# gchq/annchor

Measured on AMD Instinct MI355X. Metric: knn_graph_builds_per_s (1 / Annchor.fit() wall-clock; BASELINE: k-NN graph build time + recall@k), higher is better.
Workload: dtype int32 bit-vectors (Levenshtein) + f64 (bounds/regression/selection); 1 GPU; load_strings Levenshtein N=1600 n_anchors=15 k=25 p_work=0.12 niters=2; parallelism=one GPU

## Files before the change

annchor_amd/csrc/select.hip:

```cpp
#include "common.h"
#include "rowsel.h"
#include "selstate.h"

__global__ __launch_bounds__(ROW_THREADS) void k_row_thresh(const int64_t *__restrict__ Iptr, RowSrc src, uint32_t k,
                                                           double *__restrict__ thresh, int cap)
{
    __shared__ RowSelShared sh;
    __shared__ RowCand rc;
    extern __shared__ __attribute__((aligned(16))) unsigned char dyn_rt[];
    uint64_t *keys = reinterpret_cast<uint64_t *>(dyn_rt);
    const int64_t i = row_of_block(gridDim.x);
    const int64_t b = Iptr[i];
    const int len = (int)(Iptr[i + 1] - b);
    if (len <= 0) { if (threadIdx.x == 0) thresh[i] = -INFINITY; return; }
    const RowView rv = row_view(src, i, b);
    const uint32_t kk = k >= (uint32_t)len ? (uint32_t)len - 1 : k;
    {
        const int cnt = row_candidates(rc, len, (int)kk + 1, [&](int s) { return ann_key_asc(rv.val(s)); }, [](int) { return true; },
                                       [](int, uint64_t, bool) {});
        const int cnts = cnt > (int)kk ? row_cand_shrink(rc, cnt, (int)kk + 1, src.shrink_min) : -1;
        if (cnts > (int)kk) {
            for (int e = threadIdx.x; e < cnts; e += ROW_THREADS) {
                const uint64_t ke = rc.key[e];
                uint32_t less = 0, leq = 0;
// ... 601 lines not shown
__host__ __device__ __forceinline__ unsigned long long ann_tie_scramble(int64_t p)
{
    return ((unsigned long long)p * 0x9E3779B97F4A7C15ull) >> 11;
}

#define TIE_HB 12
#define TIE_BINS (1 << TIE_HB)
#define TIE_SHIFT (53 - TIE_HB)
#define TIE_U 8
__global__ __launch_bounds__(256) void k_tie_hist(const double *__restrict__ prob, int64_t n, CutState *__restrict__ cs,
                                                 uint32_t *__restrict__ ghist )
{
    __shared__ uint32_t h[2][TIE_BINS];
    __shared__ unsigned long long acc[4];
    for (int t = threadIdx.x; t < 2 * TIE_BINS; t += 256) (&h[0][0])[t] = 0;
    if (threadIdx.x < 4) acc[threadIdx.x] = 0;
    __syncthreads();
    const double t1 = cs->t1, t5 = cs->t5;
    const bool need1 = !cs->all1, need5 = !cs->all5;
    unsigned long long g1 = 0, g5 = 0, n1 = 0, n5 = 0;
    const int64_t stride = (int64_t)gridDim.x * blockDim.x * TIE_U;
    for (int64_t p0 = (int64_t)blockIdx.x * blockDim.x * TIE_U + threadIdx.x; p0 < n; p0 += stride) {
        double v[TIE_U];
#pragma unroll
        for (int e = 0; e < TIE_U; ++e) v[e] = ann_ldc(prob, p0 + (int64_t)e * blockDim.x, n);
#pragma unroll
        for (int e = 0; e < TIE_U; ++e) {
            const int64_t p = p0 + (int64_t)e * blockDim.x;
            if (p >= n || !(v[e] >= 0.0)) continue;
            g1 += v[e] > t1;
            g5 += v[e] > t5;
            const bool m1 = need1 && v[e] == t1, m5 = need5 && v[e] == t5;
            if (m1 || m5) {
                const uint32_t bin = (uint32_t)(ann_tie_scramble(p) >> TIE_SHIFT);
                if (m1) { atomicAdd(&h[0][bin], 1u); ++n1; }
                if (m5) { atomicAdd(&h[1][bin], 1u); ++n5; }
            }
        }
    }
#pragma unroll
    for (int off = 32; off > 0; off >>= 1) {
        g1 += __shfl_xor(g1, off); g5 += __shfl_xor(g5, off); n1 += __shfl_xor(n1, off); n5 += __shfl_xor(n5, off);
    }
    if ((threadIdx.x & 63) == 0) { atomicAdd(&acc[0], g1); atomicAdd(&acc[1], g5); atomicAdd(&acc[2], n1); atomicAdd(&acc[3], n5); }
    __syncthreads();
    for (int t = threadIdx.x; t < 2 * TIE_BINS; t += 256) {
        const uint32_t c = (&h[0][0])[t];
        if (c) atomicAdd(&ghist[t], c);
    }
    if (threadIdx.x == 0) {
        if (acc[0]) atomicAdd((unsigned long long *)&cs->tie_gt1, acc[0]);
        if (acc[1]) atomicAdd((unsigned long long *)&cs->tie_gt5, acc[1]);
        if (acc[2]) atomicAdd((unsigned long long *)&cs->tie_n1, acc[2]);
        if (acc[3]) atomicAdd((unsigned long long *)&cs->tie_n5, acc[3]);
    }
}

__global__ __launch_bounds__(1024) void k_tie_pick(CutState *__restrict__ cs, uint32_t *__restrict__ ghist)
{
    __shared__ unsigned long long wsum[16];
    const int lane = threadIdx.x & 63, wave = threadIdx.x >> 6;
    for (int q = 0; q < 2; ++q) {
        const bool all = q == 0 ? cs->all1 : cs->all5;
        const long long cnt = q == 0 ? cs->tie_n1 : cs->tie_n5;
        const long long e = q == 0 ? cs->K1 - cs->tie_gt1 : cs->K5 - cs->tie_gt5;
        uint32_t *h = ghist + q * TIE_BINS;
        constexpr int PER = TIE_BINS / 1024;
        unsigned long long c[PER], mine = 0;
#pragma unroll
        for (int j = 0; j < PER; ++j) { c[j] = h[threadIdx.x * PER + j]; h[threadIdx.x * PER + j] = 0; mine += c[j]; }
        unsigned long long inc = mine;
#pragma unroll
        for (int off = 1; off < 64; off <<= 1) { const unsigned long long up = __shfl_up(inc, off); if (lane >= off) inc += up; }
        __syncthreads();
        if (lane == 63) wsum[wave] = inc;
        __syncthreads();
        unsigned long long before = inc - mine;
        for (int w2 = 0; w2 < wave; ++w2) before += wsum[w2];
        if (threadIdx.x == 0) {
            unsigned long long rk = ~0ull;
            long long bin = -1;
            if (!all && e < cnt) { if (e <= 0) rk = 0ull; else bin = -2; }
            if (q == 0) { cs->rk1 = rk; cs->tie_bin1 = bin; } else { cs->rk5 = rk; cs->tie_bin5 = bin; }
        }
        __syncthreads();
        if (!all && e < cnt && e > 0 && (long long)before < e && (long long)(before + mine) >= e) {
            long long accb = (long long)before;
#pragma unroll
            for (int j = 0; j < PER; ++j) {
                if (accb < e && accb + (long long)c[j] >= e) {
                    if (q == 0) { cs->tie_bin1 = threadIdx.x * PER + j; cs->tie_rem1 = e - accb; cs->tie_len1 = (long long)c[j]; }
                    else { cs->tie_bin5 = threadIdx.x * PER + j; cs->tie_rem5 = e - accb; cs->tie_len5 = (long long)c[j]; }
                }
                accb += (long long)c[j];
            }
        }
        __syncthreads();
    }
}

#define TIE_LCAP 1024
__global__ __launch_bounds__(256) void k_tie_collect(const double *__restrict__ prob, int64_t n, CutState *__restrict__ cs,
                                                    unsigned long long *__restrict__ list1, unsigned long long *__restrict__ list5,
                                                    long long cap)
{
    __shared__ unsigned long long lbuf[2][TIE_LCAP];
    __shared__ uint32_t lcnt[2];
    __shared__ unsigned long long lbase[2];
    const long long b1 = cs->tie_bin1, b5 = cs->tie_bin5;
    if (b1 < 0 && b5 < 0) return;
    if (threadIdx.x < 2) lcnt[threadIdx.x] = 0;
    __syncthreads();
    const double t1 = cs->t1, t5 = cs->t5;
    auto put = [&](int q, unsigned long long kk) {
        const uint32_t o = atomicAdd(&lcnt[q], 1u);
        if (o < TIE_LCAP) lbuf[q][o] = kk;
        else {
            const unsigned long long g = atomicAdd((unsigned long long *)(q == 0 ? &cs->tie_got1 : &cs->tie_got5), 1ull);
            if ((long long)g < cap) (q == 0 ? list1 : list5)[g] = kk;
        }
    };
    const int64_t stride = (int64_t)gridDim.x * blockDim.x * TIE_U;
    for (int64_t p0 = (int64_t)blockIdx.x * blockDim.x * TIE_U + threadIdx.x; p0 < n; p0 += stride) {
        double v[TIE_U];
#pragma unroll
        for (int e = 0; e < TIE_U; ++e) v[e] = ann_ldc(prob, p0 + (int64_t)e * blockDim.x, n);
#pragma unroll
        for (int e = 0; e < TIE_U; ++e) {
            const int64_t p = p0 + (int64_t)e * blockDim.x;
            if (p >= n || !(v[e] >= 0.0)) continue;
            const bool m1 = b1 >= 0 && v[e] == t1, m5 = b5 >= 0 && v[e] == t5;
            if (m1 || m5) {
                const unsigned long long kk = ann_tie_scramble(p);
                const long long bin = (long long)(kk >> TIE_SHIFT);
                if (m1 && bin == b1) put(0, kk);
                if (m5 && bin == b5) put(1, kk);
            }
        }
    }
    __syncthreads();
    if (threadIdx.x < 2) {
        const uint32_t m = min(lcnt[threadIdx.x], (uint32_t)TIE_LCAP);
        lbase[threadIdx.x] = m ? atomicAdd((unsigned long long *)(threadIdx.x == 0 ? &cs->tie_got1 : &cs->tie_got5), (unsigned long long)m) : 0ull;
    }
    __syncthreads();
    for (int q = 0; q < 2; ++q) {
        const uint32_t m = min(lcnt[q], (uint32_t)TIE_LCAP);
        unsigned long long *list = q == 0 ? list1 : list5;
        for (uint32_t t = threadIdx.x; t < m; t += blockDim.x)
            if ((long long)(lbase[q] + t) < cap) list[lbase[q] + t] = lbuf[q][t];
    }
}

__global__ __launch_bounds__(1024) void k_tie_select(CutState *__restrict__ cs, const unsigned long long *__restrict__ list1,
                                                    const unsigned long long *__restrict__ list5, long long cap)
{
    __shared__ uint32_t hist[256];
    __shared__ unsigned long long prefix_s;
    __shared__ long long krem_s;
    for (int q = 0; q < 2; ++q) {
        const long long bin = q == 0 ? cs->tie_bin1 : cs->tie_bin5;
        if (bin < 0) continue;
        const long long cnt = q == 0 ? cs->tie_len1 : cs->tie_len5;
        const long long e = q == 0 ? cs->tie_rem1 : cs->tie_rem5;
        const unsigned long long *list = q == 0 ? list1 : list5;
        unsigned long long rk = 0ull;
        if (cnt > cap) { if (threadIdx.x == 0) cs->tie_overflow = 1; }
        else {
            if (threadIdx.x == 0) { prefix_s = 0; krem_s = e - 1; }
            __syncthreads();
            for (int pass = 1; pass < 8; ++pass) {
                const int shift = 56 - 8 * pass;
                const unsigned long long himask = ~0ull << (shift + 8);
                if (threadIdx.x < 256) hist[threadIdx.x] = 0;
                __syncthreads();
                const unsigned long long pre = prefix_s;
                for (long long t = threadIdx.x; t < cnt; t += 1024) {
                    const unsigned long long kk = list[t];
                    if ((kk & himask) == pre) atomicAdd(&hist[(uint32_t)(kk >> shift) & 0xffu], 1u);
                }
                __syncthreads();
                if (threadIdx.x < 64) {
                    uint32_t c4[4], s4 = 0;
#pragma unroll
                    for (int j = 0; j < 4; ++j) { c4[j] = hist[threadIdx.x * 4 + j]; s4 += c4[j]; }
                    uint32_t inc = s4;
#pragma unroll
                    for (int off = 1; off < 64; off <<= 1) { const uint32_t up = __shfl_up(inc, off); if ((int)threadIdx.x >= off) inc += up; }
                    long long k = krem_s;
                    long long acc4 = (long long)(inc - s4);
                    if (acc4 <= k && k < acc4 + (long long)s4) {
#pragma unroll
                        for (int j = 0; j < 4; ++j) {
                            if (acc4 <= k && k < acc4 + (long long)c4[j]) {
                                prefix_s = pre | ((unsigned long long)(threadIdx.x * 4 + j) << shift);
                                krem_s = k - acc4;
                            }
                            acc4 += c4[j];
                        }
                    }
                }
                __syncthreads();
            }
            rk = prefix_s;
        }
        if (threadIdx.x == 0) { if (q == 0) cs->rk1 = rk; else cs->rk5 = rk; }
        __syncthreads();
    }
}

__global__ void k_tie_flags(const double *__restrict__ prob, int64_t n, double t, uint8_t *__restrict__ flag, double *__restrict__ scr)
{
    const int64_t p = (int64_t)blockIdx.x * blockDim.x + threadIdx.x;
    if (p < n) {
        flag[p] = prob[p] == t ? 1 : 0;
        scr[p] = (double)ann_tie_scramble(p);
    }
}

__device__ __forceinline__ int cut_class(double v, double t, unsigned long long rk, const double *RA, int64_t p)
{
    if (v > t) return 2;
    if (v != t) return 0;
    if (rk == ~0ull) return 2;
    const unsigned long long kk = ann_tie_scramble(p);
    return kk < rk ? 2 : (kk == rk ? 1 : 0);
}

__global__ __launch_bounds__(CP_THREADS) void k_cut_count(const double *__restrict__ prob, const double *__restrict__ RA, int64_t n,
                                                         const CutState *__restrict__ cs, uint32_t *__restrict__ blk, int nsub)
{
    __shared__ uint32_t acc[4];
    if (threadIdx.x < 4) acc[threadIdx.x] = 0;
    __syncthreads();
    const double t1 = cs->t1, t5 = cs->t5;
    const unsigned long long rk1 = cs->rk1, rk5 = cs->rk5;
    uint32_t g1 = 0, q1 = 0, g5 = 0, q5 = 0;
    for (int sub = 0; sub < nsub; ++sub) {
        const int64_t base = ((int64_t)blockIdx.x * nsub + sub) * CP_SUBTILE;
        if (base >= n) break;
        double v[CP_ITEMS];
#pragma unroll
        for (int k = 0; k < CP_ITEMS; ++k) v[k] = ann_ldc(prob, base + (int64_t)k * CP_THREADS + threadIdx.x, n);
#pragma unroll
        for (int k = 0; k < CP_ITEMS; ++k) {
            const int64_t p = base + (int64_t)k * CP_THREADS + threadIdx.x;
            if (p < n && v[k] >= 0.0) {
                const int c1 = cut_class(v[k], t1, rk1, RA, p), c5 = cut_class(v[k], t5, rk5, RA, p);
                g1 += c1 == 2; q1 += c1 == 1; g5 += c5 == 2; q5 += c5 == 1;
            }
        }
    }
    unsigned long long pk = (unsigned long long)g1 | ((unsigned long long)q1 << 16) | ((unsigned long long)g5 << 32) |
                            ((unsigned long long)q5 << 48);
#pragma unroll
    for (int off = 32; off > 0; off >>= 1) pk += __shfl_xor(pk, off);
    if ((threadIdx.x & 63) == 0) {
        atomicAdd(&acc[0], (uint32_t)(pk & 0xffff)); atomicAdd(&acc[1], (uint32_t)((pk >> 16) & 0xffff));
        atomicAdd(&acc[2], (uint32_t)((pk >> 32) & 0xffff)); atomicAdd(&acc[3], (uint32_t)(pk >> 48));
    }
    __syncthreads();
    if (threadIdx.x < 4) blk[(size_t)blockIdx.x * 4 + threadIdx.x] = acc[threadIdx.x];
}

#define CS_THREADS 1024
#define CS_ITEMS 4
__global__ __launch_bounds__(CS_THREADS) void k_cut_scan(const uint32_t *__restrict__ blk, int nb, CutState *__restrict__ cs,
                                                        int64_t *__restrict__ off)
{
    __shared__ unsigned long long wsum[CS_THREADS / 64];
    const int lane = threadIdx.x & 63, wave = threadIdx.x >> 6;
    auto block_scan = [&](unsigned long long v, unsigned long long *total) -> unsigned long long {
        unsigned long long inc = v;
#pragma unroll
        for (int o = 1; o < 64; o <<= 1) { unsigned long long x = __shfl_up(inc, o); if (lane >= o) inc += x; }
        __syncthreads();
        if (lane == 63) wsum[wave] = inc;
        __syncthreads();
        unsigned long long base = 0, tot = 0;
        for (int w = 0; w < CS_THREADS / 64; ++w) { const unsigned long long x = wsum[w]; if (w < wave) base += x; tot += x; }
        *total = tot;
        return base + inc - v;
    };
    const uint4 *blk4 = reinterpret_cast<const uint4 *>(blk);
    unsigned long long g = 0;
    for (int t0 = threadIdx.x; t0 < nb; t0 += CS_THREADS * CS_ITEMS) {
        uint4 b[CS_ITEMS];
#pragma unroll
        for (int e = 0; e < CS_ITEMS; ++e) b[e] = ann_ldc(blk4, t0 + e * CS_THREADS, nb);
#pragma unroll
        for (int e = 0; e < CS_ITEMS; ++e)
            if (t0 + e * CS_THREADS < nb) g += (unsigned long long)b[e].x | ((unsigned long long)b[e].z << 32);
    }
    unsigned long long T;
    block_scan(g, &T);
    const int64_t T1 = (int64_t)(T & 0xffffffffull), T5 = (int64_t)(T >> 32);
    const int64_t e1 = cs->all1 ? (1ll << 62) : cs->K1 - T1;
    const int64_t e5 = cs->all5 ? (1ll << 62) : cs->K5 - T5;
    const bool both_all = cs->all1 && cs->all5;
    unsigned long long c_eq = 0, c_out = 0;
    for (int base = 0; base < nb; base += CS_THREADS * CS_ITEMS) {
        const int t0 = base + threadIdx.x * CS_ITEMS;
        uint4 b[CS_ITEMS];
#pragma unroll
        for (int e = 0; e < CS_ITEMS; ++e) {
            b[e] = ann_ldc(blk4, t0 + e, nb);
            if (t0 + e >= nb) b[e] = make_uint4(0, 0, 0, 0);
        }
        unsigned long long eqs = 0;
#pragma unroll
        for (int e = 0; e < CS_ITEMS; ++e) eqs += (unsigned long long)b[e].y | ((unsigned long long)b[e].w << 32);
        unsigned long long tot;
        unsigned long long ex = c_eq + block_scan(eqs, &tot);
        c_eq += tot;
        int64_t p1[CS_ITEMS], p5[CS_ITEMS];
        unsigned long long outv[CS_ITEMS], outs = 0;
#pragma unroll
        for (int e = 0; e < CS_ITEMS; ++e) {
            p1[e] = (int64_t)(ex & 0xffffffffull);
            p5[e] = (int64_t)(ex >> 32);
            const int64_t eq1 = b[e].y, eq5 = b[e].w;
            const int64_t take1 = min(eq1, max((int64_t)0, e1 - p1[e]));
            const int64_t take5 = min(eq5, max((int64_t)0, e5 - p5[e]));
            const int64_t ncand = (int64_t)b[e].x + take1;
            const int64_t nbig = (int64_t)b[e].z + take5;
            const int64_t nnext = both_all ? nbig : nbig - ncand;
            outv[e] = (unsigned long long)ncand | ((unsigned long long)nnext << 32);
            outs += outv[e];
            ex += (unsigned long long)eq1 | ((unsigned long long)eq5 << 32);
        }
        unsigned long long exo = c_out + block_scan(outs, &tot);
        c_out += tot;
#pragma unroll
        for (int e = 0; e < CS_ITEMS; ++e) {
            if (t0 + e < nb) {
                int64_t *o = off + (size_t)(t0 + e) * 4;
                o[0] = p1[e]; o[1] = p5[e]; o[2] = (int64_t)(exo & 0xffffffffull); o[3] = (int64_t)(exo >> 32);
            }
            exo += outv[e];
        }
    }
    if (threadIdx.x == 0) { cs->e1 = e1; cs->e5 = e5; cs->ncand = (int64_t)(c_out & 0xffffffffull); cs->nnext = (int64_t)(c_out >> 32); }
}

__global__ __launch_bounds__(CP_THREADS) void k_cut_emit(const double *__restrict__ prob, const double *__restrict__ RA, int64_t n,
                                                        const CutState *__restrict__ cs, const int64_t *__restrict__ off,
                                                        int32_t *__restrict__ cand, int32_t *__restrict__ next, int nsub)
{
    __shared__ uint32_t wsum[CP_THREADS / 64];
    const double t1 = cs->t1, t5 = cs->t5;
    const unsigned long long rk1 = cs->rk1, rk5 = cs->rk5;
    const int64_t e1 = cs->e1, e5 = cs->e5;
    const bool both_all = cs->all1 && cs->all5;
    auto scan2 = [&](uint32_t a, uint32_t b, uint32_t *ea, uint32_t *eb, uint32_t *ta, uint32_t *tb) {
        uint32_t tot;
        const uint32_t packed = row_block_scan((a << 16) | b, wsum, &tot);
        __syncthreads();
        *ea = packed >> 16;
        *eb = packed & 0xffffu;
        *ta = tot >> 16;
        *tb = tot & 0xffffu;
    };
    int64_t R1 = off[(size_t)blockIdx.x * 4], R5 = off[(size_t)blockIdx.x * 4 + 1];
    int64_t WC = off[(size_t)blockIdx.x * 4 + 2], WN = off[(size_t)blockIdx.x * 4 + 3];
    for (int sub = 0; sub < nsub; ++sub) {
        const int64_t sbase = ((int64_t)blockIdx.x * nsub + sub) * CP_SUBTILE;
        if (sbase >= n) break;
        const int64_t base = sbase + (int64_t)threadIdx.x * CP_ITEMS;
        double v[CP_ITEMS];
        int8_t k1[CP_ITEMS], k5[CP_ITEMS];
        uint32_t q1 = 0, q5 = 0;
#pragma unroll
        for (int k = 0; k < CP_ITEMS; ++k) {
            v[k] = (base + k < n) ? prob[base + k] : -1.0;
            k1[k] = k5[k] = 0;
            if (v[k] >= 0.0) {
                k1[k] = (int8_t)cut_class(v[k], t1, rk1, RA, base + k);
                k5[k] = (int8_t)cut_class(v[k], t5, rk5, RA, base + k);
                q1 += k1[k] == 1; q5 += k5[k] == 1;
            }
        }
        uint32_t x1, x5, tq1, tq5;
        scan2(q1, q5, &x1, &x5, &tq1, &tq5);
        int64_t r1 = R1 + x1, r5 = R5 + x5;
        uint8_t fc[CP_ITEMS], fn[CP_ITEMS];
        uint32_t nc = 0, nn = 0;
#pragma unroll
        for (int k = 0; k < CP_ITEMS; ++k) {
            bool c1 = false, c5 = false;
            if (v[k] >= 0.0) {
                c1 = k1[k] == 2 || (k1[k] == 1 && r1 < e1);
                c5 = k5[k] == 2 || (k5[k] == 1 && r5 < e5);
                r1 += k1[k] == 1;
                r5 += k5[k] == 1;
            }
            fc[k] = c1;
            fn[k] = both_all ? c5 : (c5 && !c1);
            nc += fc[k];
            nn += fn[k];
        }
        uint32_t oc, on, tc, tn;
        scan2(nc, nn, &oc, &on, &tc, &tn);
        int64_t wc = WC + oc, wn = WN + on;
#pragma unroll
        for (int k = 0; k < CP_ITEMS; ++k) {
            if (fc[k]) cand[wc++] = (int32_t)(base + k);
            if (fn[k]) next[wn++] = (int32_t)(base + k);
        }
        R1 += tq1; R5 += tq5; WC += tc; WN += tn;
    }
}

#define SEL_ERR_OFF 256
#define SEL_STATE_BYTES (SEL_ERR_OFF + 256)
static_assert(sizeof(CutState) <= SEL_ERR_OFF, "the error flag sits behind the cut state");
static inline int32_t *gn_err_ptr(annchor_ctx *c) { return reinterpret_cast<int32_t *>(c->sel_state.as<char>() + SEL_ERR_OFF); }
size_t ann_sel_state_bytes() { return SEL_STATE_BYTES; }
#define GN_BATCH 8

static int select_stage_a(annchor_ctx *c, int32_t n_neighbors, int32_t nmin)
{
    const int64_t n = c->n, nx = c->nx;
    c->gn_pending = false;
    ANN_TRY(ann_reserve(c, c->thresh, sizeof(double) * (size_t)nx));
    ANN_CHECK_HIP(c, hipEventRecord(c->call_a, c->stream));
    RowSrc rsrc;
    ANN_TRY(ann_transpose_columns(c, &rsrc));
    {
        ProfScope ps(c, "row_kth_threshold", (double)n * 24.0);
        int cap = 2;
        if (!rsrc.T) ANN_TRY(row_pick_cap(c, k_row_thresh, nx, nx, 0, &cap));
        ANN_TRY(row_lds_prepare(c, k_row_thresh, (size_t)cap * 8));
        k_row_thresh<<<(int)nx, ROW_THREADS, (size_t)cap * 8, c->stream>>>(c->Iptr.as<int64_t>(), rsrc, (uint32_t)n_neighbors,
                                                                         c->thresh.as<double>(), cap);
    }
    if (nmin > 0) {
        const int L = nmin + 1;
        ANN_REQUIRE(c, L <= 1024, ANNCHOR_ELIMIT, "nmin=%d too large", nmin);
        ANN_TRY(ann_reserve(c, c->gl_val, sizeof(double) * (size_t)nx * L));
        ANN_TRY(ann_reserve(c, c->gl_pos, sizeof(int32_t) * (size_t)nx * L * 3));
        ANN_TRY(ann_reserve(c, c->gl_cnt, sizeof(int32_t) * (size_t)nx));
        ANN_TRY(ann_reserve(c, c->gl_ncomp, sizeof(int32_t) * (size_t)nx));
        ANN_TRY(ann_reserve(c, c->sel_state, SEL_STATE_BYTES));
        if (!c->gn_err_clean) {
            ANN_CHECK_HIP(c, hipMemsetAsync(gn_err_ptr(c), 0, 4, c->stream));
        }
        c->gn_err_clean = false;
        {
            ProfScope ps(c, "guarantee_nmin_lists", (double)n * 26.0);
            const size_t tail = (((size_t)L * 12) + 15) & ~(size_t)15;
            int cap = 2;
            if (!rsrc.T) ANN_TRY(row_pick_cap(c, k_gn_lists, nx, nx, tail, &cap));
            ANN_TRY(row_lds_prepare(c, k_gn_lists, (size_t)cap * 8 + tail));
            k_gn_lists<<<(int)nx, ROW_THREADS, (size_t)cap * 8 + tail, c->stream>>>(
                c->Iptr.as<int64_t>(), rsrc, c->ij.as<int2>(), L,
                c->gl_val.as<double>(), c->gl_pos.as<int32_t>(), c->gl_pos.as<int32_t>() + (size_t)nx * L,
                c->gl_cnt.as<int32_t>(), c->gl_ncomp.as<int32_t>(), cap);
        }
        const size_t sweep_lds = (size_t)nx * (((size_t)L + 31) / 32 * 4 + 4);
        const size_t ring_lds = sweep_lds + 2 * (size_t)GN_B * L * 20 + 64 * 20 + 4 * GN_B * 4 + 64 + 16;
        const char *gn_env = getenv("ANNCHOR_GN_SWEEP");
        if (!gn_env || strcmp(gn_env, "sequential") != 0) {
            ProfScope ps(c, "guarantee_nmin_sweep", (double)nx * L * 21.0);
            int32_t *oth = c->gl_pos.as<int32_t>() + (size_t)nx * L, *twin = oth + (size_t)nx * L;
            k_gn_twin<<<ann_blocks(nx * L, 256), 256, 0, c->stream>>>(nx, L, c->gl_pos.as<int32_t>(), oth,
                                                                     c->gl_cnt.as<int32_t>(), twin);
            const int Lw = (L + 31) / 32;
            const size_t mask_bytes = sizeof(uint32_t) * (size_t)nx * Lw, mout_bytes = sizeof(int32_t) * (size_t)nx;

            ANN_TRY(ann_reserve(c, c->gn_state, 2 * mask_bytes + 3 * mout_bytes + sizeof(int32_t) * GN_BATCH));
            uint32_t *masks[2] = {c->gn_state.as<uint32_t>(), c->gn_state.as<uint32_t>() + (size_t)nx * Lw};
            int32_t *mout[3];
            for (int q = 0; q < 3; ++q) mout[q] = reinterpret_cast<int32_t *>(c->gn_state.as<char>() + 2 * mask_bytes + q * mout_bytes);
            int32_t *changed = reinterpret_cast<int32_t *>(c->gn_state.as<char>() + 2 * mask_bytes + 3 * mout_bytes);
            ANN_CHECK_HIP(c, hipMemsetAsync(c->gn_state.p, 0, 2 * mask_bytes + 3 * mout_bytes + sizeof(int32_t) * GN_BATCH, c->stream));
            int round = 0;
            for (int q = 0; q < GN_BATCH; ++q, ++round)
                k_gn_round<<<ann_blocks(nx * 64, 256), 256, 0, c->stream>>>(
                    nx, nmin, L, Lw, c->gl_val.as<double>(), oth, twin, c->gl_cnt.as<int32_t>(), c->gl_ncomp.as<int32_t>(),
                    masks[round & 1], masks[(round + 1) & 1], mout[round % 3], mout[(round + 1) % 3], mout[(round + 2) % 3],
                    changed + q, gn_err_ptr(c));
            c->gn_pending = true; c->gn_round = round; c->gn_L = L;
        } else if (L <= GN_LMAX && ring_lds <= 156 * 1024) {
            ProfScope ps(c, "guarantee_nmin_sweep", (double)nx * L * 21.0);
            int32_t *oth = c->gl_pos.as<int32_t>() + (size_t)nx * L, *twin = oth + (size_t)nx * L;
            k_gn_twin<<<ann_blocks(nx * L, 256), 256, 0, c->stream>>>(nx, L, c->gl_pos.as<int32_t>(), oth,
                                                                     c->gl_cnt.as<int32_t>(), twin);
            ANN_CHECK_HIP(c, hipFuncSetAttribute((const void *)k_gn_sweep_ring, hipFuncAttributeMaxDynamicSharedMemorySize,
                                                 (int)ring_lds));
            k_gn_sweep_ring<<<1, 256, ring_lds, c->stream>>>(nx, nmin, L, c->gl_val.as<double>(), c->gl_pos.as<int32_t>(), oth, twin,
                                                            c->gl_cnt.as<int32_t>(), c->gl_ncomp.as<int32_t>(),
                                                            c->RA.as<double>(), gn_err_ptr(c));
        } else if (sweep_lds <= 150 * 1024) {
            ProfScope ps(c, "guarantee_nmin_sweep", (double)nx * L * 21.0);
            int32_t *oth = c->gl_pos.as<int32_t>() + (size_t)nx * L, *twin = oth + (size_t)nx * L;
            k_gn_twin<<<ann_blocks(nx * L, 256), 256, 0, c->stream>>>(nx, L, c->gl_pos.as<int32_t>(), oth,
                                                                     c->gl_cnt.as<int32_t>(), twin);
            if (sweep_lds > 64 * 1024)
                ANN_CHECK_HIP(c, hipFuncSetAttribute((const void *)k_gn_sweep_lds, hipFuncAttributeMaxDynamicSharedMemorySize,
                                                     (int)sweep_lds));
            k_gn_sweep_lds<<<1, 64, sweep_lds, c->stream>>>(nx, nmin, L, c->gl_val.as<double>(), c->gl_pos.as<int32_t>(), oth,
                                                           twin, c->gl_cnt.as<int32_t>(), c->gl_ncomp.as<int32_t>(),
                                                           c->RA.as<double>(), gn_err_ptr(c));
        } else {
            ANN_TRY(ann_reserve(c, c->marked, (size_t)n));
            ANN_TRY(ann_reserve(c, c->markcount, sizeof(int32_t) * (size_t)nx));
            ANN_CHECK_HIP(c, hipMemsetAsync(c->marked.p, 0, (size_t)n, c->stream));
            ANN_CHECK_HIP(c, hipMemsetAsync(c->markcount.p, 0, sizeof(int32_t) * (size_t)nx, c->stream));
            ProfScope ps(c, "guarantee_nmin_sweep", (double)nx * L * 13.0);
            k_gn_sequential<<<1, 64, 0, c->stream>>>(nx, nmin, L, c->gl_val.as<double>(), c->gl_pos.as<int32_t>(),
                                                    c->gl_cnt.as<int32_t>(), c->gl_ncomp.as<int32_t>(), c->ij.as<int2>(),
                                                    c->RA.as<double>(), c->marked.as<uint8_t>(), c->markcount.as<int32_t>(),
                                                    gn_err_ptr(c));
        }
    }
    return ANNCHOR_OK;
}

static int select_stage_finish(annchor_ctx *c)
{
    if (!c->gn_pending) return ANNCHOR_OK;
    const int64_t nx = c->nx;
    const int L = c->gn_L, Lw = (L + 31) / 32, nmin = L - 1;
    const size_t mask_bytes = sizeof(uint32_t) * (size_t)nx * Lw, mout_bytes = sizeof(int32_t) * (size_t)nx;
    uint32_t *masks[2] = {c->gn_state.as<uint32_t>(), c->gn_state.as<uint32_t>() + (size_t)nx * Lw};
    int32_t *mout[3];
    for (int q = 0; q < 3; ++q) mout[q] = reinterpret_cast<int32_t *>(c->gn_state.as<char>() + 2 * mask_bytes + q * mout_bytes);
    int32_t *changed = reinterpret_cast<int32_t *>(c->gn_state.as<char>() + 2 * mask_bytes + 3 * mout_bytes);
    int32_t *oth = c->gl_pos.as<int32_t>() + (size_t)nx * L, *twin = oth + (size_t)nx * L;
    int round = c->gn_round;
    for (;;) {
        int32_t h_changed[GN_BATCH];
        ANN_TRY(ann_d2h(c, h_changed, changed, sizeof h_changed));
        if (h_changed[GN_BATCH - 1] == 0) break;
        ANN_REQUIRE(c, round <= (int)nx + GN_BATCH, ANNCHOR_EHIP, "guarantee_nmin rounds did not settle");
        ANN_CHECK_HIP(c, hipMemsetAsync(changed, 0, sizeof(int32_t) * GN_BATCH, c->stream));
        for (int q = 0; q < GN_BATCH; ++q, ++round)
            k_gn_round<<<ann_blocks(nx * 64, 256), 256, 0, c->stream>>>(
                nx, nmin, L, Lw, c->gl_val.as<double>(), oth, twin, c->gl_cnt.as<int32_t>(), c->gl_ncomp.as<int32_t>(),
                masks[round & 1], masks[(round + 1) & 1], mout[round % 3], mout[(round + 1) % 3], mout[(round + 2) % 3],
                changed + q, gn_err_ptr(c));
    }
    k_gn_apply<<<ann_blocks(nx * L, 256), 256, 0, c->stream>>>(nx, L, Lw, c->gl_pos.as<int32_t>(), c->gl_cnt.as<int32_t>(),
                                                              masks[round & 1], c->RA.as<double>());
    ANN_CHECK_HIP(c, hipGetLastError());
    c->gn_pending = false;
    return ANNCHOR_OK;
}

size_t ann_tie_hist_bytes() { return sizeof(uint32_t) * 2 * TIE_BINS; }

extern "C" int annchor_select_prepare(annchor_ctx *c, int32_t n_neighbors, int32_t nmin)
{
    if (!c) return ANNCHOR_EINVAL;
    ANN_REQUIRE(c, c->have_RA, ANNCHOR_EINVAL, "RefineApprox not initialised");
    ANN_REQUIRE(c, n_neighbors >= 1 && nmin >= 0, ANNCHOR_EINVAL, "bad selection parameters");
    ANN_CHECK_HIP(c, hipSetDevice(c->device));
    ANN_TRY(select_stage_a(c, n_neighbors, nmin));
    c->sel_prepared = true; c->sel_k = n_neighbors; c->sel_nmin = nmin;
    return ANNCHOR_OK;
}

extern "C" int annchor_select_candidates(annchor_ctx *c, int32_t n_neighbors, int32_t nmin, const double *errs,
                                         const int64_t *err_ptr, int32_t nlabels, int64_t n_refine, int32_t lookahead,
                                         int64_t *n_cand, int64_t *n_next)
{
    if (!c || (errs && !err_ptr) || !n_cand || !n_next) return ANNCHOR_EINVAL;
    ANN_REQUIRE(c, c->have_RA, ANNCHOR_EINVAL, "RefineApprox not initialised");
    const bool dev_errs = errs == nullptr;
    ANN_REQUIRE(c, !dev_errs || (c->errs_on_device && nlabels == c->model_nb), ANNCHOR_ESTATE,
                "no device-resident residual lists for %d labels (annchor_fit_errors_device)", nlabels);
    ANN_REQUIRE(c, nlabels >= 1 && nlabels <= 255, ANNCHOR_ELIMIT, "1..255 error labels supported");
    ANN_REQUIRE(c, n_neighbors >= 1 && lookahead >= 1 && n_refine >= 0, ANNCHOR_EINVAL, "bad selection parameters");
    if (!dev_errs)
        for (int b = 0; b < nlabels; ++b)
            ANN_REQUIRE(c, err_ptr[b + 1] > err_ptr[b], ANNCHOR_ESTATE, "error bin %d has no samples", b);
    ANN_CHECK_HIP(c, hipSetDevice(c->device));
    const int64_t n = c->n, nx = c->nx;
    if (!(c->sel_prepared && c->sel_k == n_neighbors && c->sel_nmin == nmin)) ANN_TRY(select_stage_a(c, n_neighbors, nmin));
    c->sel_prepared = false;
    ANN_TRY(select_stage_finish(c));
    (void)nx;
    const int64_t nerr = dev_errs ? 2 * c->nsamp + 64 : err_ptr[nlabels];
    if (!dev_errs) {
        ANN_TRY(ann_reserve(c, c->errs, sizeof(double) * (size_t)nerr));
        ANN_TRY(ann_reserve(c, c->errptr, sizeof(int64_t) * (size_t)(MAXBINS > nlabels ? MAXBINS + 1 : nlabels + 1)));
        ANN_TRY(ann_h2d(c, c->errs.p, errs, sizeof(double) * (size_t)nerr));
        ANN_TRY(ann_h2d(c, c->errptr.p, err_ptr, sizeof(int64_t) * (size_t)(nlabels + 1)));
        c->errs_on_device = false; c->model_cache_valid = false;
    }
    {
        const int64_t lds_entries = dev_errs ? c->nsamp + 64 : nerr;
        const int in_lds = lds_entries * 8 <= 60 * 1024;
        const size_t dyn = in_lds ? (size_t)lds_entries * 8 : 0;
        int blocks = min(ann_blocks(n, 256 * 8), c->prop.multiProcessorCount * 8);
        ProfScope ps(c, "ecdf_probability", (double)n * 26.0);
        static const long long index_min = getenv("ANNCHOR_ECDF_INDEX_MIN") ? atoll(getenv("ANNCHOR_ECDF_INDEX_MIN")) : (4ll << 20);
        EcdfIndex *index = nullptr;
        uint32_t *table = nullptr;
        if (n >= index_min && nlabels > 0 && nerr > 0 && nerr < (1ll << 29)) {
            const size_t idx_bytes = (sizeof(EcdfIndex) * (size_t)nlabels + 15) & ~(size_t)15;
            ANN_TRY(ann_reserve(c, c->ecdf_index, idx_bytes + sizeof(uint32_t) * (size_t)(2 * nerr + nlabels + 1)));
            index = c->ecdf_index.as<EcdfIndex>();
            table = reinterpret_cast<uint32_t *>(c->ecdf_index.as<char>() + idx_bytes);
            k_ecdf_index<<<nlabels, 256, 0, c->stream>>>(c->errs.as<double>(), c->errptr.as<int64_t>(), index, table);
        }
        k_prob<<<blocks, 256, dyn, c->stream>>>(n, c->ij.as<int2>(), c->thresh.as<double>(), c->RA.as<double>(),
                                               c->ncm.as<uint8_t>(), c->label.as<uint8_t>(), c->errs.as<double>(),
                                               c->errptr.as<int64_t>(), nlabels, in_lds ? (int)lds_entries : 0, c->prob.as<double>(), n >= ANN_STREAM_MIN_PAIRS,
                                               index, table);
    }
    ANN_CHECK_HIP(c, hipGetLastError());
    int64_t n_unc = 0;
    ANN_TRY(annchor_count_uncomputed(c, &n_unc));
    CutState cs;
    memset(&cs, 0, sizeof cs);
    cs.K1 = n_refine;
    cs.K5 = n_refine * (int64_t)lookahead;
    cs.all1 = n_refine >= n_unc;
    cs.all5 = cs.all1 || cs.K5 >= n_unc;
    cs.t1 = cs.t5 = INFINITY;
    const unsigned long long *d_cut_prefix = nullptr;
    const int *d_cut_unfinished = nullptr;
    int64_t cut_ks[2];
    int cut_nk = 0;
    auto cut_values_waiting = [&]() -> int {
        double tv[2];
        ANN_TRY(ann_kth_smallest(c, c->prob.as<double>(), c->ncm.as<uint8_t>(), n, cut_ks, cut_nk, tv));
        int q = 0;
        if (!cs.all1) cs.t1 = tv[q++];
        if (!cs.all5) cs.t5 = tv[q++];
        return ANNCHOR_OK;
    };
    if (cs.all1) cs.t1 = -1.0;
    if (cs.all5) cs.t5 = -1.0;
    if (n_refine == 0) { cs.all1 = cs.all5 = 0; cs.t1 = cs.t5 = INFINITY; cs.K1 = cs.K5 = 0; }
    const int nsub = cp_nsub(n);
    const int nb = ann_blocks(n, (int64_t)CP_SUBTILE * nsub);
    ANN_TRY(ann_reserve(c, c->sel_state, SEL_STATE_BYTES));
    ANN_TRY(ann_reserve(c, c->blk_cnt, sizeof(uint32_t) * 4 * (size_t)nb));
    ANN_TRY(ann_reserve(c, c->blk_off, sizeof(int64_t) * 4 * (size_t)nb));
    const int64_t maxc = cs.all1 ? n_unc : cs.K1, maxn = cs.all5 ? n_unc : cs.K5;
    ANN_TRY(ann_reserve(c, c->cand, sizeof(int32_t) * (size_t)(maxc + 1)));
    ANN_TRY(ann_reserve(c, c->next, sizeof(int32_t) * (size_t)(maxn + 1)));
    cs.rk1 = cs.rk5 = ~0ull;
    if (n_refine > 0 && !(cs.all1 && cs.all5)) {
        if (!cs.all1) cut_ks[cut_nk++] = n_unc - cs.K1;
        if (!cs.all5) cut_ks[cut_nk++] = n_unc - cs.K5;
        if (!getenv("ANNCHOR_CUT_WAIT")) {
            Sel2Epilogue ep;
            memset(&ep, 0, sizeof ep);
            ep.kind = 2; ep.cs = c->sel_state.as<CutState>(); ep.cs_init = cs; ep.need1 = !cs.all1; ep.need5 = !cs.all5;
            ep.force_redo = getenv("ANNCHOR_CUT_FORCE_REDO") ? 1 : 0;
            ANN_TRY(ann_kth_async(c, c->prob.as<double>(), c->ncm.as<uint8_t>(), n, cut_ks, cut_nk, &d_cut_prefix, &d_cut_unfinished, &ep));
        }
        if (!d_cut_prefix) ANN_TRY(cut_values_waiting());
    }
    const CutState cs_in = cs;
    if (!d_cut_prefix) ANN_TRY(ann_h2d(c, c->sel_state.p, &cs, sizeof cs));
    const bool ties = n_refine > 0 && !(cs.all1 && cs.all5);
    ANN_TRY(ann_reserve(c, c->tie_lists, sizeof(unsigned long long) * 2 * TIE_CAP));
    unsigned long long *tl1 = c->tie_lists.as<unsigned long long>(), *tl5 = tl1 + TIE_CAP;
    auto split = [&]() {
        ProfScope ps(c, "topk_split_compact", (double)n * 16.0 + (double)(maxc + maxn) * 4.0);
        k_cut_count<<<nb, CP_THREADS, 0, c->stream>>>(c->prob.as<double>(), c->RA.as<double>(), n, c->sel_state.as<CutState>(),
                                                     c->blk_cnt.as<uint32_t>(), nsub);
        k_cut_scan<<<1, CS_THREADS, 0, c->stream>>>(c->blk_cnt.as<uint32_t>(), nb, c->sel_state.as<CutState>(), c->blk_off.as<int64_t>());
        k_cut_emit<<<nb, CP_THREADS, 0, c->stream>>>(c->prob.as<double>(), c->RA.as<double>(), n, c->sel_state.as<CutState>(),
                                                    c->blk_off.as<int64_t>(), c->cand.as<int32_t>(), c->next.as<int32_t>(), nsub);
    };
    auto tie_groups = [&]() -> int {
        ProfScope ps(c, "topk_tie_groups", (double)n * 8.0);
        const int tb = (int)std::min<int64_t>(ann_blocks(n, 256 * TIE_U), (int64_t)c->prop.multiProcessorCount * 3);
        const char *cap_env = getenv("ANNCHOR_TIE_CAP");
        const long long cap = cap_env ? std::min<long long>(TIE_CAP, std::max<long long>(1, atoll(cap_env))) : TIE_CAP;
        ANN_TRY(ann_reserve(c, c->tie_hist, sizeof(uint32_t) * 2 * TIE_BINS));
        if (c->tie_hist_clean != c->tie_hist.p) {
            ANN_CHECK_HIP(c, hipMemsetAsync(c->tie_hist.p, 0, sizeof(uint32_t) * 2 * TIE_BINS, c->stream));
            c->tie_hist_clean = c->tie_hist.p;
        }
        k_tie_hist<<<tb, 256, 0, c->stream>>>(c->prob.as<double>(), n, c->sel_state.as<CutState>(), c->tie_hist.as<uint32_t>());
        k_tie_pick<<<1, 1024, 0, c->stream>>>(c->sel_state.as<CutState>(), c->tie_hist.as<uint32_t>());
        k_tie_collect<<<tb, 256, 0, c->stream>>>(c->prob.as<double>(), n, c->sel_state.as<CutState>(), tl1, tl5, cap);
        k_tie_select<<<1, 1024, 0, c->stream>>>(c->sel_state.as<CutState>(), tl1, tl5, cap);
        return ANNCHOR_OK;
    };
    if (ties) ANN_TRY(tie_groups());
    split();
    ANN_CHECK_HIP(c, hipEventRecord(c->call_b, c->stream));
    c->call_timed = true;
    ANN_CHECK_HIP(c, hipGetLastError());
    if (nmin > 0) {
        unsigned char both[SEL_ERR_OFF + 4];
        ANN_TRY(ann_d2h(c, both, c->sel_state.p, sizeof both));
        int32_t e = 0;
        memcpy(&cs, both, sizeof cs);
        memcpy(&e, both + SEL_ERR_OFF, 4);
        c->gn_err_clean = e == 0;
        ANN_REQUIRE(c, e == 0, ANNCHOR_ESTATE, "guarantee_nmin: a row has fewer not-computed candidates than it must refine");
    } else {
        ANN_TRY(ann_d2h(c, &cs, c->sel_state.p, sizeof cs));
    }
    if (d_cut_prefix) {
        ann_kth_async_done(c);
        if (cs.sel_unfinished) {
            cs = cs_in;
            ANN_TRY(cut_values_waiting());
            ANN_TRY(ann_h2d(c, c->sel_state.p, &cs, sizeof cs));
            if (ties) ANN_TRY(tie_groups());
            split();
            ANN_CHECK_HIP(c, hipGetLastError());
            ANN_TRY(ann_d2h(c, &cs, c->sel_state.p, sizeof cs));
        }
    }
    if (cs.tie_overflow) {
        ANN_TRY(ann_reserve(c, c->marked, (size_t)n));
        for (int q = 0; q < 2; ++q) {
            const bool all = q == 0 ? cs.all1 : cs.all5;
            const int64_t cnt = q == 0 ? cs.tie_n1 : cs.tie_n5, e = q == 0 ? cs.K1 - cs.tie_gt1 : cs.K5 - cs.tie_gt5;
            unsigned long long rk = ~0ull;
            if (!all && e < cnt) {
                if (e <= 0) rk = 0ull;
                else {
                    ANN_TRY(ann_reserve(c, c->colT, sizeof(double) * (size_t)n));
                    k_tie_flags<<<ann_blocks(n, 256), 256, 0, c->stream>>>(c->prob.as<double>(), n, q == 0 ? cs.t1 : cs.t5, c->marked.as<uint8_t>(),
                                                                          c->colT.as<double>());
                    int64_t kq = e - 1;
                    double rv = 0;
                    ANN_TRY(ann_kth_smallest(c, c->colT.as<double>(), c->marked.as<uint8_t>(), n, &kq, 1, &rv));
                    rk = (unsigned long long)rv;
                }
            }
            if (q == 0) cs.rk1 = rk; else cs.rk5 = rk;
        }
        cs.tie_overflow = 0; cs.e1 = cs.e5 = 0; cs.ncand = cs.nnext = 0;
        ANN_TRY(ann_h2d(c, c->sel_state.p, &cs, sizeof cs));
        split();
        ANN_CHECK_HIP(c, hipGetLastError());
        ANN_TRY(ann_d2h(c, &cs, c->sel_state.p, sizeof cs));
    }
    c->ncand = cs.ncand;
    c->n_unc = n_unc;
    c->cand_marked = false;
    c->nnext = cs.nnext;
    *n_cand = cs.ncand;
    *n_next = cs.nnext;
    return ANNCHOR_OK;
}

__global__ void k_mark_candidates(const int32_t *__restrict__ pos, int64_t m, uint8_t *__restrict__ ncm)
{
    int64_t t = (int64_t)blockIdx.x * blockDim.x + threadIdx.x;
    if (t < m) ncm[pos[t]] = 0;
}

extern "C" int annchor_mark_candidates(annchor_ctx *c)
{
    if (!c) return ANNCHOR_EINVAL;
    ANN_REQUIRE(c, c->have_RA, ANNCHOR_EINVAL, "RefineApprox not initialised");
    if (c->ncand == 0 || c->cand_marked) return ANNCHOR_OK;
    ANN_CHECK_HIP(c, hipSetDevice(c->device));
    k_mark_candidates<<<ann_blocks(c->ncand, 256), 256, 0, c->stream>>>(c->cand.as<int32_t>(), c->ncand, c->ncm.as<uint8_t>());
    ANN_CHECK_HIP(c, hipGetLastError());
    if (c->n_unc >= 0) c->n_unc -= c->ncand;
    c->cand_marked = true; c->sel_prepared = false;
    return ANNCHOR_OK;
}

extern "C" int annchor_park_refine(annchor_ctx *c, int32_t action)
{
    if (!c || (action != 1 && action != 2)) return ANNCHOR_EINVAL;
    if (action == 1) { c->park_refine = true; return ANNCHOR_OK; }
    if (!c->park_refine) return ANNCHOR_OK;
    c->park_refine = false;
    return annchor_refine_candidates(c);
}

extern "C" int annchor_refine_candidates(annchor_ctx *c)
{
    if (!c) return ANNCHOR_EINVAL;
    ANN_REQUIRE(c, c->have_RA, ANNCHOR_EINVAL, "RefineApprox not initialised");
    ANN_REQUIRE(c, c->metric != ANNCHOR_METRIC_NONE, ANNCHOR_EINVAL, "no device metric bound to this context");
    if (c->ncand == 0) return ANNCHOR_OK;
    ANN_CHECK_HIP(c, hipSetDevice(c->device));
    PairSource src;
    src.ij = c->ij.as<int2>();
    src.idx = c->cand.as<int32_t>();
    src.n = c->ncand;
    ANN_CHECK_HIP(c, hipEventRecord(c->call_a, c->stream));
    ANN_TRY(ann_metric_launch(c, src, nullptr, c->RA.as<double>(), c->ncm.as<uint8_t>()));
    ANN_CHECK_HIP(c, hipEventRecord(c->call_b, c->stream));
    c->call_timed = true;
    ANN_CHECK_HIP(c, hipGetLastError());
    if (c->n_unc >= 0 && !c->cand_marked) c->n_unc -= c->ncand;
    c->cand_marked = true; c->sel_prepared = false;
    return ANNCHOR_OK;
}

__global__ void k_write_refined(const int32_t *__restrict__ pos, const double *__restrict__ v, int64_t m,
                                double *__restrict__ RA, uint8_t *__restrict__ ncm)
{
    int64_t t = (int64_t)blockIdx.x * blockDim.x + threadIdx.x;
    if (t < m) { RA[pos[t]] = v[t]; ncm[pos[t]] = 0; }
}

extern "C" int annchor_set_refined(annchor_ctx *c, const double *exact, int64_t n_cand)
{
    if (!c || (n_cand > 0 && !exact)) return ANNCHOR_EINVAL;
    ANN_REQUIRE(c, c->have_RA, ANNCHOR_EINVAL, "RefineApprox not initialised");
    ANN_REQUIRE(c, n_cand == c->ncand, ANNCHOR_EINVAL, "expected %lld refined values, got %lld", (long long)c->ncand,
                (long long)n_cand);
    if (n_cand == 0) return ANNCHOR_OK;
    ANN_CHECK_HIP(c, hipSetDevice(c->device));
    ANN_TRY(ann_reserve(c, c->stage_in, sizeof(double) * (size_t)n_cand));
    ANN_TRY(ann_h2d(c, c->stage_in.p, exact, sizeof(double) * (size_t)n_cand));
    k_write_refined<<<ann_blocks(n_cand, 256), 256, 0, c->stream>>>(c->cand.as<int32_t>(), c->stage_in.as<double>(), n_cand,
                                                                   c->RA.as<double>(), c->ncm.as<uint8_t>());
    ANN_CHECK_HIP(c, hipGetLastError());
    if (c->n_unc >= 0 && !c->cand_marked) c->n_unc -= n_cand;
    c->cand_marked = true; c->sel_prepared = false;
    return ANNCHOR_OK;
}
```

Baseline: 364.6 graphs/s.

## Fold tie-select and cut-scan into count/emit kernels to cut launches

When the number of cut tiles is small, the single-block tie-select kernel is folded into k_cut_count and the single-block cut-scan kernel into k_cut_emit. Each block redundantly recomputes the tie rank, using a brute-force pairwise rank when the tie list fits in one block, and recomputes the block-offset scan itself. This removes two serialized tiny launches per split, at the cost of duplicated work in every block and extra shared memory and registers. An environment variable can restore the separate path.

```diff
diff --git a/annchor_amd/csrc/select.hip b/annchor_amd/csrc/select.hip
--- a/annchor_amd/csrc/select.hip
+++ b/annchor_amd/csrc/select.hip
@@ -777,6 +777,47 @@
     }
 }
 
+__device__ __forceinline__ unsigned long long tie_radix_rank(const unsigned long long *__restrict__ list, long long cnt, long long e,
+                                                             uint32_t *hist , unsigned long long *prefix_s, long long *krem_s)
+{
+    if (threadIdx.x == 0) { *prefix_s = 0; *krem_s = e - 1; }
+    __syncthreads();
+    for (int pass = 1; pass < 8; ++pass) {
+        const int shift = 56 - 8 * pass;
+        const unsigned long long himask = ~0ull << (shift + 8);
+        if (threadIdx.x < 256) hist[threadIdx.x] = 0;
+        __syncthreads();
+        const unsigned long long pre = *prefix_s;
+        for (long long t = threadIdx.x; t < cnt; t += blockDim.x) {
+            const unsigned long long kk = list[t];
+            if ((kk & himask) == pre) atomicAdd(&hist[(uint32_t)(kk >> shift) & 0xffu], 1u);
+        }
+        __syncthreads();
+        if (threadIdx.x < 64) {
+            uint32_t c4[4], s4 = 0;
+#pragma unroll
+            for (int j = 0; j < 4; ++j) { c4[j] = hist[threadIdx.x * 4 + j]; s4 += c4[j]; }
+            uint32_t inc = s4;
+#pragma unroll
+            for (int off = 1; off < 64; off <<= 1) { const uint32_t up = __shfl_up(inc, off); if ((int)threadIdx.x >= off) inc += up; }
+            long long k = *krem_s;
+            long long acc4 = (long long)(inc - s4);
+            if (acc4 <= k && k < acc4 + (long long)s4) {
+#pragma unroll
+                for (int j = 0; j < 4; ++j) {
+                    if (acc4 <= k && k < acc4 + (long long)c4[j]) {
+                        *prefix_s = pre | ((unsigned long long)(threadIdx.x * 4 + j) << shift);
+                        *krem_s = k - acc4;
+                    }
+                    acc4 += c4[j];
+                }
+            }
+        }
+        __syncthreads();
+    }
+    return *prefix_s;
+}
+
 __global__ __launch_bounds__(1024) void k_tie_select(CutState *__restrict__ cs, const unsigned long long *__restrict__ list1,
                                                     const unsigned long long *__restrict__ list5, long long cap)
 {
@@ -791,46 +832,47 @@
         const unsigned long long *list = q == 0 ? list1 : list5;
         unsigned long long rk = 0ull;
         if (cnt > cap) { if (threadIdx.x == 0) cs->tie_overflow = 1; }
+        else rk = tie_radix_rank(list, cnt, e, hist, &prefix_s, &krem_s);
+        if (threadIdx.x == 0) { if (q == 0) cs->rk1 = rk; else cs->rk5 = rk; }
+        __syncthreads();
+    }
+}
+
+#define TIE_FOLD_KEYS CP_THREADS
+__device__ __forceinline__ void tie_select_folded(CutState *__restrict__ cs, const unsigned long long *__restrict__ list1,
+                                                  const unsigned long long *__restrict__ list5, long long cap,
+                                                  unsigned long long *rk1, unsigned long long *rk5)
+{
+    __shared__ unsigned long long keys[TIE_FOLD_KEYS];
+    __shared__ uint32_t hist[256];
+    __shared__ unsigned long long prefix_s;
+    __shared__ long long krem_s;
+    for (int q = 0; q < 2; ++q) {
+        const long long bin = q == 0 ? cs->tie_bin1 : cs->tie_bin5;
+        unsigned long long rk;
+        if (bin < 0) rk = q == 0 ? cs->rk1 : cs->rk5;
         else {
-            if (threadIdx.x == 0) { prefix_s = 0; krem_s = e - 1; }
+            const long long cnt = q == 0 ? cs->tie_len1 : cs->tie_len5;
+            const long long e = q == 0 ? cs->tie_rem1 : cs->tie_rem5;
+            const unsigned long long *list = q == 0 ? list1 : list5;
+            rk = 0ull;
+            if (cnt > cap) { if (blockIdx.x == 0 && threadIdx.x == 0) cs->tie_overflow = 1; }
+            else if (cnt <= TIE_FOLD_KEYS) {
+                const bool have = (long long)threadIdx.x < cnt;
+                const unsigned long long mine = have ? list[threadIdx.x] : 0ull;
+                if (have) keys[threadIdx.x] = mine;
+                if (threadIdx.x == 0) prefix_s = 0ull;
+                __syncthreads();
+                long long lt = 0, le = 0;
+                for (int j = 0; j < (int)cnt; ++j) { const unsigned long long o = keys[j]; lt += o < mine; le += o <= mine; }
+                if (have && lt < e && e <= le) prefix_s = mine;
+                __syncthreads();
+                rk = prefix_s;
+            } else rk = tie_radix_rank(list, cnt, e, hist, &prefix_s, &krem_s);
+            if (blockIdx.x == 0 && threadIdx.x == 0) { if (q == 0) cs->rk1 = rk; else cs->rk5 = rk; }
             __syncthreads();
-            for (int pass = 1; pass < 8; ++pass) {
-                const int shift = 56 - 8 * pass;
-                const unsigned long long himask = ~0ull << (shift + 8);
-                if (threadIdx.x < 256) hist[threadIdx.x] = 0;
-                __syncthreads();
-                const unsigned long long pre = prefix_s;
-                for (long long t = threadIdx.x; t < cnt; t += 1024) {
-                    const unsigned long long kk = list[t];
-                    if ((kk & himask) == pre) atomicAdd(&hist[(uint32_t)(kk >> shift) & 0xffu], 1u);
-                }
-                __syncthreads();
-                if (threadIdx.x < 64) {
-                    uint32_t c4[4], s4 = 0;
-#pragma unroll
-                    for (int j = 0; j < 4; ++j) { c4[j] = hist[threadIdx.x * 4 + j]; s4 += c4[j]; }
-                    uint32_t inc = s4;
-#pragma unroll
-                    for (int off = 1; off < 64; off <<= 1) { const uint32_t up = __shfl_up(inc, off); if ((int)threadIdx.x >= off) inc += up; }
-                    long long k = krem_s;
-                    long long acc4 = (long long)(inc - s4);
-                    if (acc4 <= k && k < acc4 + (long long)s4) {
-#pragma unroll
-                        for (int j = 0; j < 4; ++j) {
-                            if (acc4 <= k && k < acc4 + (long long)c4[j]) {
-                                prefix_s = pre | ((unsigned long long)(threadIdx.x * 4 + j) << shift);
-                                krem_s = k - acc4;
-                            }
-                            acc4 += c4[j];
-                        }
-                    }
-                }
-                __syncthreads();
-            }
-            rk = prefix_s;
-        }
-        if (threadIdx.x == 0) { if (q == 0) cs->rk1 = rk; else cs->rk5 = rk; }
-        __syncthreads();
+        }
+        if (q == 0) *rk1 = rk; else *rk5 = rk;
     }
 }
 
@@ -853,13 +895,17 @@
 }
 
 __global__ __launch_bounds__(CP_THREADS) void k_cut_count(const double *__restrict__ prob, const double *__restrict__ RA, int64_t n,
-                                                         const CutState *__restrict__ cs, uint32_t *__restrict__ blk, int nsub)
+                                                         CutState *__restrict__ cs, uint32_t *__restrict__ blk, int nsub,
+                                                         const unsigned long long *__restrict__ list1 ,
+                                                         const unsigned long long *__restrict__ list5, long long cap)
 {
     __shared__ uint32_t acc[4];
     if (threadIdx.x < 4) acc[threadIdx.x] = 0;
     __syncthreads();
     const double t1 = cs->t1, t5 = cs->t5;
-    const unsigned long long rk1 = cs->rk1, rk5 = cs->rk5;
+    unsigned long long rk1, rk5;
+    if (list1) tie_select_folded(cs, list1, list5, cap, &rk1, &rk5);
+    else { rk1 = cs->rk1; rk5 = cs->rk5; }
     uint32_t g1 = 0, q1 = 0, g5 = 0, q5 = 0;
     for (int sub = 0; sub < nsub; ++sub) {
         const int64_t base = ((int64_t)blockIdx.x * nsub + sub) * CP_SUBTILE;
@@ -968,14 +1014,94 @@
     if (threadIdx.x == 0) { cs->e1 = e1; cs->e5 = e5; cs->ncand = (int64_t)(c_out & 0xffffffffull); cs->nnext = (int64_t)(c_out >> 32); }
 }
 
+#define CUT_FOLD_TILES (CP_THREADS * 4)
+__device__ __forceinline__ void cut_scan_folded(const uint32_t *__restrict__ blk, int nb, CutState *__restrict__ cs, int64_t *e1o,
+                                                int64_t *e5o, int64_t off4[4])
+{
+    __shared__ unsigned long long wsum2[CP_THREADS / 64];
+    __shared__ int64_t mine_s[4];
+    const int lane = threadIdx.x & 63, wave = threadIdx.x >> 6;
+    auto block_scan = [&](unsigned long long v, unsigned long long *total) -> unsigned long long {
+        unsigned long long inc = v;
+#pragma unroll
+        for (int o = 1; o < 64; o <<= 1) { unsigned long long x = __shfl_up(inc, o); if (lane >= o) inc += x; }
+        __syncthreads();
+        if (lane == 63) wsum2[wave] = inc;
+        __syncthreads();
+        unsigned long long base = 0, tot = 0;
+        for (int w = 0; w < CP_THREADS / 64; ++w) { const unsigned long long x = wsum2[w]; if (w < wave) base += x; tot += x; }
+        *total = tot;
+        return base + inc - v;
+    };
+    const uint4 *blk4 = reinterpret_cast<const uint4 *>(blk);
+    const int t0 = threadIdx.x * 4;
+    uint4 b[4];
+#pragma unroll
+    for (int e = 0; e < 4; ++e) {
+        b[e] = ann_ldc(blk4, t0 + e, nb);
+        if (t0 + e >= nb) b[e] = make_uint4(0, 0, 0, 0);
+    }
+    unsigned long long g = 0, eqs = 0;
+#pragma unroll
+    for (int e = 0; e < 4; ++e) {
+        g += (unsigned long long)b[e].x | ((unsigned long long)b[e].z << 32);
+        eqs += (unsigned long long)b[e].y | ((unsigned long long)b[e].w << 32);
+    }
+    unsigned long long T, tot;
+    block_scan(g, &T);
+    const int64_t T1 = (int64_t)(T & 0xffffffffull), T5 = (int64_t)(T >> 32);
+    const int64_t e1 = cs->all1 ? (1ll << 62) : cs->K1 - T1;
+    const int64_t e5 = cs->all5 ? (1ll << 62) : cs->K5 - T5;
+    const bool both_all = cs->all1 && cs->all5;
+    unsigned long long ex = block_scan(eqs, &tot);
+    int64_t p1[4], p5[4];
+    unsigned long long outv[4], outs = 0;
+#pragma unroll
+    for (int e = 0; e < 4; ++e) {
+        p1[e] = (int64_t)(ex & 0xffffffffull);
+        p5[e] = (int64_t)(ex >> 32);
+        const int64_t eq1 = b[e].y, eq5 = b[e].w;
+        const int64_t take1 = min(eq1, max((int64_t)0, e1 - p1[e]));
+        const int64_t take5 = min(eq5, max((int64_t)0, e5 - p5[e]));
+        const int64_t ncand = (int64_t)b[e].x + take1;
+        const int64_t nbig = (int64_t)b[e].z + take5;
+        const int64_t nnext = both_all ? nbig : nbig - ncand;
+        outv[e] = (unsigned long long)ncand | ((unsigned long long)nnext << 32);
+        outs += outv[e];
+        ex += (unsigned long long)eq1 | ((unsigned long long)eq5 << 32);
+    }
+    unsigned long long exo = block_scan(outs, &tot);
+#pragma unroll
+    for (int e = 0; e < 4; ++e) {
+        if (t0 + e == (int)blockIdx.x) {
+            mine_s[0] = p1[e]; mine_s[1] = p5[e]; mine_s[2] = (int64_t)(exo & 0xffffffffull); mine_s[3] = (int64_t)(exo >> 32);
+        }
+        exo += outv[e];
+    }
+    if (blockIdx.x == 0 && threadIdx.x == 0) {
+        cs->e1 = e1; cs->e5 = e5; cs->ncand = (int64_t)(tot & 0xffffffffull); cs->nnext = (int64_t)(tot >> 32);
+    }
+    __syncthreads();
+#pragma unroll
+    for (int q = 0; q < 4; ++q) off4[q] = mine_s[q];
+    *e1o = e1; *e5o = e5;
+}
+
 __global__ __launch_bounds__(CP_THREADS) void k_cut_emit(const double *__restrict__ prob, const double *__restrict__ RA, int64_t n,
-                                                        const CutState *__restrict__ cs, const int64_t *__restrict__ off,
-                                                        int32_t *__restrict__ cand, int32_t *__restrict__ next, int nsub)
+                                                        CutState *__restrict__ cs, const int64_t *__restrict__ off,
+                                                        int32_t *__restrict__ cand, int32_t *__restrict__ next, int nsub,
+                                                        const uint32_t *__restrict__ blk , int nb)
 {
     __shared__ uint32_t wsum[CP_THREADS / 64];
     const double t1 = cs->t1, t5 = cs->t5;
     const unsigned long long rk1 = cs->rk1, rk5 = cs->rk5;
-    const int64_t e1 = cs->e1, e5 = cs->e5;
+    int64_t e1, e5, off4[4];
+    if (blk) cut_scan_folded(blk, nb, cs, &e1, &e5, off4);
+    else {
+        e1 = cs->e1; e5 = cs->e5;
+#pragma unroll
+        for (int q = 0; q < 4; ++q) off4[q] = off[(size_t)blockIdx.x * 4 + q];
+    }
     const bool both_all = cs->all1 && cs->all5;
     auto scan2 = [&](uint32_t a, uint32_t b, uint32_t *ea, uint32_t *eb, uint32_t *ta, uint32_t *tb) {
         uint32_t tot;
@@ -986,8 +1112,7 @@
         *ta = tot >> 16;
         *tb = tot & 0xffffu;
     };
-    int64_t R1 = off[(size_t)blockIdx.x * 4], R5 = off[(size_t)blockIdx.x * 4 + 1];
-    int64_t WC = off[(size_t)blockIdx.x * 4 + 2], WN = off[(size_t)blockIdx.x * 4 + 3];
+    int64_t R1 = off4[0], R5 = off4[1], WC = off4[2], WN = off4[3];
     for (int sub = 0; sub < nsub; ++sub) {
         const int64_t sbase = ((int64_t)blockIdx.x * nsub + sub) * CP_SUBTILE;
         if (sbase >= n) break;
@@ -1286,19 +1411,24 @@
     const bool ties = n_refine > 0 && !(cs.all1 && cs.all5);
     ANN_TRY(ann_reserve(c, c->tie_lists, sizeof(unsigned long long) * 2 * TIE_CAP));
     unsigned long long *tl1 = c->tie_lists.as<unsigned long long>(), *tl5 = tl1 + TIE_CAP;
-    auto split = [&]() {
+    const char *sep_env = getenv("ANNCHOR_CUT_SEPARATE");
+    const bool folded = nb <= CUT_FOLD_TILES && !(sep_env && atoi(sep_env) != 0);
+    if (c->prof_on && c->prof_mode != 2) c->prof[ann_prof_entry(c, folded ? "cut_route_folded" : "cut_route_separate")].launches += 1;
+    const char *cap_env = getenv("ANNCHOR_TIE_CAP");
+    const long long cap = cap_env ? std::min<long long>(TIE_CAP, std::max<long long>(1, atoll(cap_env))) : TIE_CAP;
+    auto split = [&](bool fold_tie_select) {
         ProfScope ps(c, "topk_split_compact", (double)n * 16.0 + (double)(maxc + maxn) * 4.0);
         k_cut_count<<<nb, CP_THREADS, 0, c->stream>>>(c->prob.as<double>(), c->RA.as<double>(), n, c->sel_state.as<CutState>(),
-                                                     c->blk_cnt.as<uint32_t>(), nsub);
-        k_cut_scan<<<1, CS_THREADS, 0, c->stream>>>(c->blk_cnt.as<uint32_t>(), nb, c->sel_state.as<CutState>(), c->blk_off.as<int64_t>());
+                                                     c->blk_cnt.as<uint32_t>(), nsub, fold_tie_select ? tl1 : nullptr, tl5, cap);
+        if (!folded)
+            k_cut_scan<<<1, CS_THREADS, 0, c->stream>>>(c->blk_cnt.as<uint32_t>(), nb, c->sel_state.as<CutState>(), c->blk_off.as<int64_t>());
         k_cut_emit<<<nb, CP_THREADS, 0, c->stream>>>(c->prob.as<double>(), c->RA.as<double>(), n, c->sel_state.as<CutState>(),
-                                                    c->blk_off.as<int64_t>(), c->cand.as<int32_t>(), c->next.as<int32_t>(), nsub);
+                                                    c->blk_off.as<int64_t>(), c->cand.as<int32_t>(), c->next.as<int32_t>(), nsub,
+                                                    folded ? c->blk_cnt.as<uint32_t>() : nullptr, nb);
     };
     auto tie_groups = [&]() -> int {
         ProfScope ps(c, "topk_tie_groups", (double)n * 8.0);
         const int tb = (int)std::min<int64_t>(ann_blocks(n, 256 * TIE_U), (int64_t)c->prop.multiProcessorCount * 3);
-        const char *cap_env = getenv("ANNCHOR_TIE_CAP");
-        const long long cap = cap_env ? std::min<long long>(TIE_CAP, std::max<long long>(1, atoll(cap_env))) : TIE_CAP;
         ANN_TRY(ann_reserve(c, c->tie_hist, sizeof(uint32_t) * 2 * TIE_BINS));
         if (c->tie_hist_clean != c->tie_hist.p) {
             ANN_CHECK_HIP(c, hipMemsetAsync(c->tie_hist.p, 0, sizeof(uint32_t) * 2 * TIE_BINS, c->stream));
@@ -1307,11 +1437,11 @@
         k_tie_hist<<<tb, 256, 0, c->stream>>>(c->prob.as<double>(), n, c->sel_state.as<CutState>(), c->tie_hist.as<uint32_t>());
         k_tie_pick<<<1, 1024, 0, c->stream>>>(c->sel_state.as<CutState>(), c->tie_hist.as<uint32_t>());
         k_tie_collect<<<tb, 256, 0, c->stream>>>(c->prob.as<double>(), n, c->sel_state.as<CutState>(), tl1, tl5, cap);
-        k_tie_select<<<1, 1024, 0, c->stream>>>(c->sel_state.as<CutState>(), tl1, tl5, cap);
+        if (!folded) k_tie_select<<<1, 1024, 0, c->stream>>>(c->sel_state.as<CutState>(), tl1, tl5, cap);
         return ANNCHOR_OK;
     };
     if (ties) ANN_TRY(tie_groups());
-    split();
+    split(ties && folded);
     ANN_CHECK_HIP(c, hipEventRecord(c->call_b, c->stream));
     c->call_timed = true;
     ANN_CHECK_HIP(c, hipGetLastError());
@@ -1333,7 +1463,7 @@
             ANN_TRY(cut_values_waiting());
             ANN_TRY(ann_h2d(c, c->sel_state.p, &cs, sizeof cs));
             if (ties) ANN_TRY(tie_groups());
-            split();
+            split(ties && folded);
             ANN_CHECK_HIP(c, hipGetLastError());
             ANN_TRY(ann_d2h(c, &cs, c->sel_state.p, sizeof cs));
         }
@@ -1360,7 +1490,7 @@
         }
         cs.tie_overflow = 0; cs.e1 = cs.e5 = 0; cs.ncand = cs.nnext = 0;
         ANN_TRY(ann_h2d(c, c->sel_state.p, &cs, sizeof cs));
-        split();
+        split(false);
         ANN_CHECK_HIP(c, hipGetLastError());
         ANN_TRY(ann_d2h(c, &cs, c->sel_state.p, sizeof cs));
     }
```

After: 367.9 graphs/s (median of 2 runs). About the same (+0.9%).
